# team-ergo-unipi/ergo_uvo

Hardware: AMD Instinct MI355X
Metric: stereo frame-pairs/sec (detect+match+pose) @1920x1080, 3k kpts (higher is better)
Workload: dtype f32+f64

## Files before the change

ergo_uvo_amd/csrc/surf.hip:

```cpp
#include "uvo_ctx.h"
#include <type_traits>
#include <string.h>
#include "uvo_math.h"
#include <algorithm>
#include <utility>
#include <vector>
#include <string>

namespace uvo {

struct ImgPair { const uint8_t* img[2]; int32_t* sum[2]; int32_t* planes[2]; int pw, pstride; int* cand_n; int* big_n; int* surv_n; };
struct AreaTab;
struct CandOut { uvo_keypoint* cand[2]; int* count; int cap; };
struct SurvOut { Survivor* list; int* count; int cap; };
static_assert(sizeof(Survivor) == 128, "a survivor record is 32 words");
struct SortArgs { const uvo_keypoint* cand[2]; const int* cand_n; uvo_keypoint* out[2]; int* out_n[2]; int* rank; int cap;
                  int4* big_par; int* big_n; int* gate_nqa; int gate_min_features; };
struct DescArgs { const uint8_t* img[2]; uvo_keypoint* kps[2]; float* desc[2]; const int* n[2]; const float* DW;
                  const int4* big_par; const int* big_n; const int* big_large; int cap;
                  const AreaTab* tabs; const int* iscale;
                  int extended;
                  const int32_t* sum[2]; const float* ori_w; int* ori_drop; };
struct LaneArgs { ImgPair ip; int32_t* part; SurvOut sv; CandOut out; SortArgs sa; DescArgs da; uint8_t* patch; const int4* big_in; int4* big_out; int* big_large; };
static const int kStripRows = 8;
// ... 707 lines not shown
    constexpr int QPR = OctTile<O, TW>::TWq / 4, kQuads = THs * QPR, kFill = UVO_FILL(kQuads, NT), kQ = NT / QPR, kR = NT % QPR;
    static_assert(STEP == 1 || STEP == 2, "tile fill handles octaves 0 and 1");
    static_assert(OctTile<O, TW>::TWq < kSumPad && STEP - OC::LO < kSumPad, "integral slack too small for the tile overshoot");
    int fidx = tid, fty = tid / QPR, fq = tid - fty * QPR;
#pragma unroll 1
    for (int i0 = 0; i0 < kQuads; i0 += NT * kFill) {
        SumQuad v[kFill];
        int dst[kFill];
#pragma unroll
        for (int u = 0; u < kFill; u++) {
            const bool in = fidx < kQuads;
            const int gy = min(max(sy0 + fty, 0), h), gx = sx0 + 4 * fq;
            v[u] = *reinterpret_cast<const SumQuad*>(gsum + (in ? gy * sw + gx : 0));
            dst[u] = in ? fty * STEP * PW + (4 / STEP) * fq : -1;
            fidx += NT; fq += kR; fty += kQ;
            if (fq >= QPR) { fq -= QPR; fty++; }
        }
#pragma unroll
        for (int u = 0; u < kFill; u++) {
            if (dst[u] < 0) continue;
            if constexpr (STEP == 1) {
                *reinterpret_cast<int4*>(stile + dst[u]) = make_int4(v[u].a, v[u].b, v[u].c, v[u].d);
            } else {
                *reinterpret_cast<int2*>(stile + dst[u]) = make_int2(v[u].a, v[u].c);
                *reinterpret_cast<int2*>(stile + dst[u] + PW) = make_int2(v[u].b, v[u].d);
            }
        }
    }
    nms_zero<TW, TH>(reinterpret_cast<unsigned*>(stile + THs * STEP * PW));
    __syncthreads();
    hess_stamp(1);
    det_layer_c<O, 1, TW, TH, NT>(stile, sdet, op, px0, py0, thr);
    det_layer_c<O, 2, TW, TH, NT>(stile, sdet, op, px0, py0, thr);
    det_layer_c<O, 3, TW, TH, NT>(stile, sdet, op, px0, py0, thr);
    __syncthreads();
    hess_stamp(2);
    nms_survivors<TW, TH, NT>(sdet, reinterpret_cast<unsigned*>(stile + THs * STEP * PW), op, thr, px0, py0, im, sv);
}
template <int O, int TW, int TH, int NT>
__global__ __launch_bounds__(NT) void k_hessian_nms_c(LaneArgs LA, int w, int h, OctavePat op, float thr)
{
    extern __shared__ __align__(16) unsigned char smem[];
    hessian_nms_c_tile<O, TW, TH, NT>(LA.ip, w, h, op, thr, LA.sv, blockIdx.x, blockIdx.y, blockIdx.z, smem);
}

template <int O, int TW, int TH, int NT>
__global__ __launch_bounds__(NT) void k_hessian_nms_p(LaneArgs LA, int w, int h, OctavePat op, float thr)
{
    __shared__ float sdet[3 * TH * TW];
    __shared__ unsigned s_list[NmsLds<TW, TH>::kWords];
    const ImgPair& ip = LA.ip; const SurvOut& sv = LA.sv;
    const int im = blockIdx.z;
    const int px0 = blockIdx.x * (TW - 2) - 1, py0 = blockIdx.y * (TH - 2) - 1;
    det_layer_p<O, 1, TW, TH, NT>(ip.planes[im], ip.pw, ip.pstride, sdet, op, px0, py0, thr);
    det_layer_p<O, 2, TW, TH, NT>(ip.planes[im], ip.pw, ip.pstride, sdet, op, px0, py0, thr);
    det_layer_p<O, 3, TW, TH, NT>(ip.planes[im], ip.pw, ip.pstride, sdet, op, px0, py0, thr);
    nms_zero<TW, TH>(s_list);
    __syncthreads();
    nms_survivors<TW, TH, NT>(sdet, s_list, op, thr, px0, py0, im, sv);
}

static const int kP23Threads = 512;
struct P23Grid { int nbx2, nb2, nbx3, nb3; };
template <class OP>
__device__ __forceinline__ void hessian_nms_p23_tile(const ImgPair& ip, const OP& op2, const OP& op3, float thr, const SurvOut& sv,
                                                     bool oct3, int bx, int by, int im, float* sdet, unsigned* s_list)
{
    constexpr int TW2 = 32, TH2 = 16, TW3 = 16, TH3 = 16;
    static_assert(TW3 * TH3 <= TW2 * TH2 && NmsLds<TW3, TH3>::kWords <= NmsLds<TW2, TH2>::kWords, "octave 3 reuses octave 2's LDS");
    if (!oct3) {
        const int px0 = bx * (TW2 - 2) - 1, py0 = by * (TH2 - 2) - 1;
        det_layers_p3<2, TW2, TH2, kP23Threads>(ip.planes[im], ip.pw, ip.pstride, sdet, op2, px0, py0, thr);
        nms_zero<TW2, TH2>(s_list);
        __syncthreads();
        hess_stamp(2);
        nms_survivors<TW2, TH2, kP23Threads>(sdet, s_list, op2, thr, px0, py0, im, sv);
    } else {
        const int px0 = bx * (TW3 - 2) - 1, py0 = by * (TH3 - 2) - 1;
        det_layers_p3<3, TW3, TH3, kP23Threads>(ip.planes[im], ip.pw, ip.pstride, sdet, op3, px0, py0, thr);
        nms_zero<TW3, TH3>(s_list);
        __syncthreads();
        hess_stamp(2);
        nms_survivors<TW3, TH3, kP23Threads>(sdet, s_list, op3, thr, px0, py0, im, sv);
    }
}
static const int kP23SdetFloats = 3 * 16 * 32;
static const int kO1TileRows = 18;
struct HessGrid { int nbx0, nb0, nbx1, nb1; P23Grid g; };
template <int TW, int TH>
__global__ __launch_bounds__(kP23Threads) void k_hessian_nms_all(LaneArgs LA, int w, int h, HessDims hd, float thr,
                                                                 const uint32_t* __restrict__ order)
{
    extern __shared__ __align__(16) unsigned char smem[];
    const ImgPair& ip = LA.ip;
    SurvOut sv = LA.sv;
    asm volatile("" : "+s"(sv.list), "+s"(sv.count), "+s"(sv.cap));
    const int im = blockIdx.y;
    const unsigned e = order[blockIdx.x];
    const int kind = e >> 30, bx = e & 0x3FFF, by = (e >> 14) & 0x3FFF;
    hess_stamp(0); hess_stamp(4, kind);
    if (kind == 0) hessian_nms_c_tile<0, TW, TH, kP23Threads>(ip, w, h, hd.o[0], thr, sv, bx, by, im, smem);
    else if (kind == 1) hessian_nms_c_tile<1, 32, kO1TileRows, kP23Threads>(ip, w, h, hd.o[1], thr, sv, bx, by, im, smem);
    else {
        float* sdet = reinterpret_cast<float*>(smem);
        hessian_nms_p23_tile(ip, hd.o[2], hd.o[3], thr, sv, kind == 3, bx, by, im, sdet, reinterpret_cast<unsigned*>(sdet + kP23SdetFloats));
    }
    hess_stamp(3);
}

__global__ __launch_bounds__(256) void k_probe_hold(int ticks)
{
    extern __shared__ int probe_lds[];
    if (threadIdx.x == 0) probe_lds[0] = ticks;
    const long long t0 = wall_clock64();
    while (wall_clock64() - t0 < ticks) __builtin_amdgcn_s_sleep(16);
}

__global__ void k_hessian_layer_debug(const int32_t* gsum, int w, int h, LayerPat lp, int step, int rows, int cols,
                                      float* det, float* trace)
{
    int j = blockIdx.x * blockDim.x + threadIdx.x, i = blockIdx.y;
    if (j >= lp.samples_j || i >= lp.samples_i) return;
    const int sw = w + 1;
    const int32_t* o = gsum + (size_t)(i * step) * sw + j * step;
    float dx, dy, dxy;
    haar_response(lp, [&](int yy, int xx) { return o[(size_t)yy * sw + xx]; }, &dx, &dy, &dxy);
    size_t pos = (size_t)(i + lp.margin) * cols + (j + lp.margin);
    det[pos] = dx * dy - 0.81f * dxy * dxy;
    trace[pos] = dx + dy;
}

__device__ __forceinline__ uint32_t ord_f32(float f)
{
    uint32_t b = __float_as_uint(f);
    return b ^ ((b >> 31) ? 0xFFFFFFFFu : 0x80000000u);
}
struct SortKey { unsigned long long k1, k2, k3; };
__device__ __forceinline__ SortKey make_sort_key(const uvo_keypoint& kp)
{
    SortKey k;
    k.k1 = ((unsigned long long)ord_f32(kp.response) << 32) | ord_f32(kp.size);
    k.k2 = ((unsigned long long)(uint32_t)kp.octave << 32) | ord_f32(kp.y);
    k.k3 = ((unsigned long long)(~ord_f32(kp.x)) << 32) | (uint32_t)(1 - kp.class_id);
    return k;
}

static const int kSmallWin = 128;
static const int kMaxWin = 740;
static const int kBigBins = 1024;
static const int kTripleWin = 246;
static const int kOrderThreads = 1024;
static const int kOrderPer = 8;
static const int kOrderCap = kOrderThreads * kOrderPer;
static const int kOrderBucketBits = 12;
static const int kOrderBuckets = 1 << kOrderBucketBits;
static const int kOrderBinsPer = kOrderBuckets / kOrderThreads;
static_assert(kOrderBuckets % kOrderThreads == 0 && kBigBins == kOrderThreads, "k_order scans kOrderBinsPer buckets and one window bin per thread");
static_assert(kOrderCap <= 65536, "bucket members are 16-bit candidate indices");

__global__ __launch_bounds__(1024) void k_big_sort(LaneArgs LA, int cap, const int* __restrict__ iscale_tab)
{
    const int4* __restrict__ in = LA.big_in; int4* __restrict__ out = LA.big_out; const int* __restrict__ big_n = LA.da.big_n; int* __restrict__ big_large = LA.big_large;
    const int im = blockIdx.x, tid = threadIdx.x;
    if (min(LA.sa.cand_n[im], cap) <= kOrderCap) return;
    const int n = min(big_n[im], cap);
    __shared__ int hist[kBigBins], scan[kBigBins];
    hist[tid] = 0;
    __syncthreads();
    for (int e = tid; e < n; e += 1024) atomicAdd(&hist[min(kBigBins - 1, max(0, kBigBins - 1 - in[im * cap + e].y))], 1);
    __syncthreads();
    int v = hist[tid];
    scan[tid] = v;
    __syncthreads();
    for (int off = 1; off < kBigBins; off <<= 1) {
        const int add = tid >= off ? scan[tid - off] : 0;
        __syncthreads();
        scan[tid] += add;
        __syncthreads();
    }
    hist[tid] = scan[tid] - v;
    if (tid == kBigBins - 1 - kTripleWin) big_large[im] = scan[tid] - v;
    __syncthreads();
    for (int e = tid; e < n; e += 1024) {
        int4 par = in[im * cap + e];
        const int pos = atomicAdd(&hist[min(kBigBins - 1, max(0, kBigBins - 1 - par.y))], 1);
        par.y |= iscale_tab[min(par.y, kMaxWin)] << 16;
        out[im * cap + pos] = par;
    }
}
static const int kSortChunk = 128;

__device__ __forceinline__ int wave_incl_scan(int v)
{
    const int lane = threadIdx.x & 63;
#pragma unroll
    for (int d = 1; d < 64; d <<= 1) { const int t = __shfl_up(v, d); if (lane >= d) v += t; }
    return v;
}

__global__ __launch_bounds__(kOrderThreads) void k_order(LaneArgs LA, const int* __restrict__ iscale_tab)
{
    const SortArgs& a = LA.sa;
    const int im = blockIdx.y, tid = threadIdx.x, lane = tid & 63, wv = tid >> 6;
    const int n = min(a.cand_n[im], a.cap);
    if (n > kOrderCap) return;
    __shared__ unsigned long long s_k1[kOrderCap];
    __shared__ unsigned short s_mem[kOrderCap];
    __shared__ int s_bin[kOrderBuckets];
    __shared__ int s_win[kBigBins];
    __shared__ int s_wave[2][kOrderThreads / 64];
    __shared__ unsigned s_lo, s_hi;
#pragma unroll
    for (int k = 0; k < kOrderBinsPer; k++) s_bin[tid * kOrderBinsPer + k] = 0;
    s_win[tid] = 0;
    if (tid == 0) { s_lo = 0xFFFFFFFFu; s_hi = 0; }
    __syncthreads();

    uvo_keypoint kp[kOrderPer];
    unsigned long long k1[kOrderPer];
    int wbin[kOrderPer];
    unsigned lo = 0xFFFFFFFFu, hi = 0;
#pragma unroll
    for (int k = 0; k < kOrderPer; k++) kp[k] = a.cand[im][min(k * kOrderThreads + tid, max(n - 1, 0))];
#pragma unroll
    for (int k = 0; k < kOrderPer; k++) {
        const int e = k * kOrderThreads + tid;
        wbin[k] = -1;
        k1[k] = make_sort_key(kp[k]).k1;
        if (e < n) {
            const unsigned r = ord_f32(kp[k].response);
            lo = min(lo, r); hi = max(hi, r);
            const float sc = kp[k].size * 1.2f / 9.0f;
            const int win_size = (int)((20 + 1) * sc);
            if (win_size > kSmallWin) { wbin[k] = min(kBigBins - 1, max(0, kBigBins - 1 - win_size)); atomicAdd(&s_win[wbin[k]], 1); }
        }
    }
#pragma unroll
    for (int d = 32; d > 0; d >>= 1) { lo = min(lo, (unsigned)__shfl_xor((int)lo, d)); hi = max(hi, (unsigned)__shfl_xor((int)hi, d)); }
    if (lane == 0) { atomicMin(&s_lo, lo); atomicMax(&s_hi, hi); }
    __syncthreads();

    lo = s_lo; hi = s_hi;
    const int bits = hi > lo ? 32 - __clz((int)(hi - lo)) : 0;
    const int sh = bits > kOrderBucketBits ? bits - kOrderBucketBits : 0;
    int bkt[kOrderPer];
#pragma unroll
    for (int k = 0; k < kOrderPer; k++) {
        const int e = k * kOrderThreads + tid;
        bkt[k] = -1;
        if (e < n) { bkt[k] = kOrderBuckets - 1 - (int)((ord_f32(kp[k].response) - lo) >> sh); atomicAdd(&s_bin[bkt[k]], 1); }
    }
    __syncthreads();

    int cnt[kOrderBinsPer], sb = 0;
#pragma unroll
    for (int k = 0; k < kOrderBinsPer; k++) { cnt[k] = s_bin[tid * kOrderBinsPer + k]; sb += cnt[k]; }
    const int wcnt = s_win[tid];
    const int ib = wave_incl_scan(sb), iw = wave_incl_scan(wcnt);
    if (lane == 63) { s_wave[0][wv] = ib; s_wave[1][wv] = iw; }
    __syncthreads();
    int xb = ib - sb, xw = iw - wcnt, wtot = 0;
    for (int v = 0; v < kOrderThreads / 64; v++) { if (v < wv) { xb += s_wave[0][v]; xw += s_wave[1][v]; } wtot += s_wave[1][v]; }
#pragma unroll
    for (int k = 0; k < kOrderBinsPer; k++) { s_bin[tid * kOrderBinsPer + k] = xb; xb += cnt[k]; }
    s_win[tid] = xw;
    if (tid == kBigBins - 1 - kTripleWin) LA.big_large[im] = xw;
    if (tid == 0) {
        a.big_n[im] = wtot;
        *a.out_n[im] = n;
        if (im == 0 && a.gate_nqa) {
            const int nL = n, nR = min(a.cand_n[1], a.cap);
            *a.gate_nqa = (nL >= a.gate_min_features && nR >= a.gate_min_features) ? nL : 0;
        }
    }
    __syncthreads();
    int slot[kOrderPer];
#pragma unroll
    for (int k = 0; k < kOrderPer; k++)
        if (bkt[k] >= 0) { slot[k] = atomicAdd(&s_bin[bkt[k]], 1); s_mem[slot[k]] = (unsigned short)(k * kOrderThreads + tid); s_k1[slot[k]] = k1[k]; }
    __syncthreads();

#pragma unroll
    for (int k = 0; k < kOrderPer; k++) {
        if (bkt[k] < 0) continue;
        const int e = k * kOrderThreads + tid;
        const int beg = bkt[k] > 0 ? s_bin[bkt[k] - 1] : 0, end = s_bin[bkt[k]];
        int rank = beg;
#pragma unroll 4
        for (int q = beg; q < end; q++) {
            const unsigned long long o1 = s_k1[q];
            rank += o1 > k1[k] ? 1 : 0;
            if (o1 == k1[k] && q != slot[k]) {
                const int f = s_mem[q];
                const SortKey mine = make_sort_key(kp[k]), o = make_sort_key(a.cand[im][f]);
                rank += (o.k2 > mine.k2 || (o.k2 == mine.k2 && (o.k3 > mine.k3 || (o.k3 == mine.k3 && f < e)))) ? 1 : 0;
            }
        }
        a.out[im][rank] = kp[k];
        if (wbin[k] >= 0) {
            const float sc = kp[k].size * 1.2f / 9.0f;
            const int win_size = (int)((20 + 1) * sc);
            const float win_offset = -(float)(win_size - 1) / 2;
            const int pos = atomicAdd(&s_win[wbin[k]], 1);
            LA.big_out[im * a.cap + pos] = make_int4(rank, win_size | (iscale_tab[min(win_size, kMaxWin)] << 16),
                                                     cv_round_f(kp[k].x + win_offset), cv_round_f(kp[k].y - win_offset));
        }
    }
}

__global__ __launch_bounds__(256) void k_rank_partial(LaneArgs LA)
{
    const SortArgs& a = LA.sa;
    const int im = blockIdx.y, tid = threadIdx.x;
    const int n = min(a.cand_n[im], a.cap);
    if (n <= kOrderCap) return;
    __shared__ SortKey tile[kSortChunk];
    __shared__ unsigned long long tile_k1[kSortChunk];
    const int nib = (n + 255) / 256, ntiles = nib * ((n + kSortChunk - 1) / kSortChunk);
    for (int t_ = blockIdx.x; t_ < ntiles; t_ += gridDim.x) {
        const int i0 = (t_ % nib) * 256, j0 = (t_ / nib) * kSortChunk;
        const int cnt = min(kSortChunk, n - j0);
        const int me = i0 + tid;
        uvo_keypoint mykp = {};
        if (me < n) mykp = a.cand[im][me];
        for (int t = tid; t < cnt; t += 256) { tile[t] = make_sort_key(a.cand[im][j0 + t]); tile_k1[t] = tile[t].k1; }
        __syncthreads();
        if (me < n) {
            const SortKey mine = make_sort_key(mykp);
            int rank = 0;
#pragma unroll 16
            for (int k = 0; k < cnt; k++) {
                const unsigned long long o1 = tile_k1[k];
                rank += o1 > mine.k1 ? 1 : 0;
                if (o1 == mine.k1) {
                    const SortKey o = tile[k];
                    rank += (o.k2 > mine.k2 || (o.k2 == mine.k2 && (o.k3 > mine.k3 || (o.k3 == mine.k3 && j0 + k < me)))) ? 1 : 0;
                }
            }
            atomicAdd(&a.rank[im * a.cap + me], rank);
        }
        __syncthreads();
    }
}

__global__ __launch_bounds__(256) void k_rank_scatter(LaneArgs LA)
{
    const SortArgs& a = LA.sa;
    const int im = blockIdx.y;
    const int n = min(a.cand_n[im], a.cap);
    if (n <= kOrderCap) return;
    const int me = blockIdx.x * 256 + threadIdx.x;
    bool big = false;
    int4 par = make_int4(0, 0, 0, 0);
    if (me < n) {
        int r = a.rank[im * a.cap + me];
        a.rank[im * a.cap + me] = 0;
        const uvo_keypoint kp = a.cand[im][me];
        a.out[im][r] = kp;
        const float sc = kp.size * 1.2f / 9.0f;
        const int win_size = (int)((20 + 1) * sc);
        if (win_size > kSmallWin) {
            const float win_offset = -(float)(win_size - 1) / 2;
            big = true;
            par = make_int4(r, win_size, cv_round_f(kp.x + win_offset), cv_round_f(kp.y - win_offset));
        }
    }
    {
        const int lane = threadIdx.x & 63;
        const unsigned long long m = __ballot(big);
        if (m != 0) {
            int base = 0;
            const int leader = __ffsll((long long)m) - 1;
            if (lane == leader) base = atomicAdd(&a.big_n[im], __popcll(m));
            base = __shfl(base, leader);
            if (big) a.big_par[im * a.cap + base + __popcll(m & ((1ull << lane) - 1))] = par;
        }
    }
    if (me == 0) *a.out_n[im] = n;
    if (me == 0 && im == 0 && a.gate_nqa) {
        const int nL = n, nR = min(a.cand_n[1], a.cap);
        *a.gate_nqa = (nL >= a.gate_min_features && nR >= a.gate_min_features) ? nL : 0;
    }
}

struct AreaTab { int sx1, sx2; float a_first, a_mid, a_last; bool has_first, has_last; };

__host__ __device__ __forceinline__ AreaTab area_tab(int dx, int ssize, double scale)
{
    AreaTab t;
    double fsx1 = dx * scale;
    double fsx2 = fsx1 + scale;
    double cellWidth = scale < ssize - fsx1 ? scale : ssize - fsx1;
    int sx1 = cv_ceil_d(fsx1), sx2 = cv_floor_d(fsx2);
    sx2 = sx2 < ssize - 1 ? sx2 : ssize - 1;
    sx1 = sx1 < sx2 ? sx1 : sx2;
    t.sx1 = sx1; t.sx2 = sx2;
    t.has_first = sx1 - fsx1 > 1e-3;
    t.a_first = (float)((sx1 - fsx1) / cellWidth);
    t.a_mid = (float)(1.0 / cellWidth);
    t.has_last = fsx2 - sx2 > 1e-3;
    double a = fsx2 - sx2; if (a > 1.) a = 1.; if (a > cellWidth) a = cellWidth;
    t.a_last = (float)(a / cellWidth);
    return t;
}

__device__ __forceinline__ uint8_t sat_u8(float v) { int iv = cv_round_f(v); return (uint8_t)(iv < 0 ? 0 : iv > 255 ? 255 : iv); }


__device__ __forceinline__ void describe_tail(const DescArgs& a, int im, int k, const int (*PATCH)[21])
{
    const int tid = threadIdx.x;
    __shared__ float DX[20][20], DY[20][20];
    __shared__ float vec[128];
    __shared__ float s_scale;
    const int dsize = a.extended ? 128 : 64;
    for (int o = tid; o < 400; o += 256) {
        int i = o / 20, j = o - i * 20;
        float dw = a.DW[o];
        float vx = (PATCH[i][j+1] - PATCH[i][j] + PATCH[i+1][j+1] - PATCH[i+1][j]) * dw;
        float vy = (PATCH[i+1][j] - PATCH[i][j] + PATCH[i+1][j+1] - PATCH[i][j+1]) * dw;
        DX[i][j] = vx; DY[i][j] = vy;
    }
    __syncthreads();
    if (tid < dsize) {
        float acc = 0.f;
        if (!a.extended) {
            int cell = tid >> 2, comp = tid & 3, ci = cell >> 2, cj = cell & 3;
            for (int y = ci * 5; y < ci * 5 + 5; y++)
                for (int x = cj * 5; x < cj * 5 + 5; x++) {
                    float t = (comp & 1) ? DY[y][x] : DX[y][x];
                    acc += (comp & 2) ? (float)fabs(t) : t;
                }
        } else {
            int cell = tid >> 3, comp = tid & 7, ci = cell >> 2, cj = cell & 3;
            for (int y = ci * 5; y < ci * 5 + 5; y++)
                for (int x = cj * 5; x < cj * 5 + 5; x++) {
                    const float tx = DX[y][x], ty = DY[y][x];
                    const float val = comp < 4 ? tx : ty, sel = comp < 4 ? ty : tx;
                    const bool take = (comp & 2) ? sel < 0 : sel >= 0;
                    if (take) acc += (comp & 1) ? (float)fabs(val) : val;
                }
        }
        vec[tid] = acc;
    }
    __syncthreads();
    if (tid == 0) {
        double square_mag = 0;
        for (int kk = 0; kk < dsize; kk++) square_mag += vec[kk] * vec[kk];
        s_scale = (float)(1. / (sqrt(square_mag) + FLT_EPSILON));
    }
    __syncthreads();
    if (tid < dsize) a.desc[im][(size_t)k * dsize + tid] = vec[tid] * s_scale;
}

static const int kTapBatch = 16;
__device__ long long* g_desc_stamps = nullptr;
__device__ __forceinline__ void desc_stamp(int im, int k, int slot, long long v = -1)
{
#if UVO_STAMPS
// ... 685 lines not shown

struct MergedGrid { int nbx0, nb0, nbx1, nb1, nb23, total; P23Grid g; };
static const int kMergedTW0 = 64, kMergedTH0 = 32, kMergedTW1 = 32;
static MergedGrid merged_grid(const OctavePat* ops)
{
    constexpr int TW0 = kMergedTW0, TH0 = kMergedTH0, TW1 = kMergedTW1, TH1 = kO1TileRows;
    MergedGrid m;
    m.nbx0 = (ops[0].cols + TW0 - 3) / (TW0 - 2); m.nb0 = m.nbx0 * ((ops[0].rows + TH0 - 3) / (TH0 - 2));
    m.nbx1 = (ops[1].cols + TW1 - 3) / (TW1 - 2); m.nb1 = m.nbx1 * ((ops[1].rows + TH1 - 3) / (TH1 - 2));
    m.g.nbx2 = (ops[2].cols + 32 - 3) / (32 - 2); m.g.nb2 = m.g.nbx2 * ((ops[2].rows + 16 - 3) / (16 - 2));
    m.g.nbx3 = (ops[3].cols + 16 - 3) / (16 - 2); m.g.nb3 = m.g.nbx3 * ((ops[3].rows + 16 - 3) / (16 - 2));
    m.nb23 = m.g.nb2 + m.g.nb3; m.total = m.nb0 + m.nb1 + m.nb23;
    return m;
}
static bool merged_launch(const Ctx* c)
{
    static const bool split_env = getenv("UVO_HESSIAN_SPLIT") != nullptr;
    return c->p.SURF_OCTAVES_NUMBER == 4 && !split_env;
}

uvo_status surf_prepare(Ctx* c, int w, int h)
{
    if (c->p.SURF_OCTAVES_NUMBER < 1 || c->p.SURF_OCTAVES_NUMBER > 4 || c->p.SURF_OCTAVES_LAYERS != 3) {
        c->err = "SURF: supported nOctaves 1..4, nOctaveLayers 3";
        return UVO_INVALID_ARG;
    }
    OctavePat ops[4];
    memset(ops, 0, sizeof(ops));
    for (int o = 0; o < c->p.SURF_OCTAVES_NUMBER; o++) make_octave(o, c->p.SURF_OCTAVES_LAYERS, w, h, &ops[o]);
    if (!c->d_octpat) UVO_HIP_TRY(c, hipMalloc(&c->d_octpat, sizeof(ops)));
    if (c->h_octpat.size() != sizeof(ops) || memcmp(c->h_octpat.data(), ops, sizeof(ops)) != 0) {
        UVO_HIP_TRY(c, hipStreamSynchronize(c->stream));
        c->h_octpat.assign(reinterpret_cast<const unsigned char*>(ops), reinterpret_cast<const unsigned char*>(ops) + sizeof(ops));
        UVO_HIP_TRY(c, hipMemcpyAsync(c->d_octpat, c->h_octpat.data(), sizeof(ops), hipMemcpyHostToDevice, c->stream));
        UVO_HIP_TRY(c, hipStreamSynchronize(c->stream));
    }
    if (!merged_launch(c)) return UVO_OK;
    const MergedGrid m = merged_grid(ops);
    const int nb0 = m.nb0, nb1 = m.nb1, nb23 = m.nb23, total = m.total;
    if (nb0 > 0x3FFF || nb1 > 0x3FFF || nb23 > 0x3FFF) { c->err = "SURF: image too large for the merged detection launch's tile table"; return UVO_INVALID_ARG; }
    const int ng[3] = { nb0, nb1, nb23 }, ngroups = total;
    if ((int)c->h_hess_order.size() != ngroups || c->hess_order_key[0] != nb0 || c->hess_order_key[1] != nb1 || c->hess_order_key[2] != nb23) {
        std::vector<std::pair<double, uint32_t>> pos;
        pos.reserve((size_t)ngroups);
        for (int k = 0; k < 3; k++) for (int i = 0; i < ng[k]; i++) {
            uint32_t e;
            if (k == 0) e = (0u << 30) | ((uint32_t)(i / m.nbx0) << 14) | (uint32_t)(i % m.nbx0);
            else if (k == 1) e = (1u << 30) | ((uint32_t)(i / m.nbx1) << 14) | (uint32_t)(i % m.nbx1);
            else if (i < m.g.nb2) e = (2u << 30) | ((uint32_t)(i / m.g.nbx2) << 14) | (uint32_t)(i % m.g.nbx2);
            else e = (3u << 30) | ((uint32_t)((i - m.g.nb2) / m.g.nbx3) << 14) | (uint32_t)((i - m.g.nb2) % m.g.nbx3);
            pos.emplace_back((i + 0.5) / ng[k] + k * 1e-9, e);
        }
        std::sort(pos.begin(), pos.end());
        c->h_hess_order.resize((size_t)ngroups);
        for (int b = 0; b < ngroups; b++) c->h_hess_order[(size_t)b] = pos[(size_t)b].second;
        UVO_HIP_TRY(c, hipStreamSynchronize(c->stream));
        if (c->d_hess_order_cap < (size_t)ngroups) {
            if (c->d_hess_order) (void)hipFree(c->d_hess_order);
            c->d_hess_order = nullptr; c->d_hess_order_cap = 0;
            UVO_HIP_TRY(c, hipMalloc(reinterpret_cast<void**>(&c->d_hess_order), sizeof(uint32_t) * (size_t)ngroups));
            c->d_hess_order_cap = (size_t)ngroups;
        }
        UVO_HIP_TRY(c, hipMemcpyAsync(c->d_hess_order, c->h_hess_order.data(), sizeof(uint32_t) * (size_t)ngroups, hipMemcpyHostToDevice, c->stream));
        UVO_HIP_TRY(c, hipStreamSynchronize(c->stream));
        c->hess_order_key[0] = nb0; c->hess_order_key[1] = nb1; c->hess_order_key[2] = nb23;
    }
    return UVO_OK;
}

uvo_status surf_detect(Ctx* c, int nimg, int gate_min_features)
{
    const int w = c->img_w, h = c->img_h;
    UVO_TRY(surf_prepare(c, w, h));
    const LaneArgs LA = lane_args(c, nimg, gate_min_features);
    UVO_TRY(surf_integral_launch(c, LA, nimg));
    const float thr = (float)c->p.SURF_MIN_HESSIAN;
    {
        OctavePat ops[4];
        memset(ops, 0, sizeof(ops));
        for (int o = 0; o < c->p.SURF_OCTAVES_NUMBER; o++) make_octave(o, c->p.SURF_OCTAVES_LAYERS, w, h, &ops[o]);
        const bool merged = merged_launch(c);
        if (merged) {
            constexpr int TW0 = kMergedTW0, TH0 = kMergedTH0, TW1 = kMergedTW1, TH1 = kO1TileRows;
            constexpr int THs0 = (TH0 - 1) * OctC<0>::STEP + (OctC<0>::HI - OctC<0>::LO) + 1, THs1 = (TH1 - 1) * OctC<1>::STEP + (OctC<1>::HI - OctC<1>::LO) + 1;
            constexpr size_t lds0 = sizeof(float) * 3 * TW0 * TH0 + sizeof(int32_t) * (size_t)THs0 * OctC<0>::STEP * OctTile<0, TW0>::PW + sizeof(unsigned) * NmsLds<TW0, TH0>::kWords;
            constexpr size_t lds1 = sizeof(float) * 3 * TW1 * TH1 + sizeof(int32_t) * (size_t)THs1 * OctC<1>::STEP * OctTile<1, TW1>::PW + sizeof(unsigned) * NmsLds<TW1, TH1>::kWords;
            constexpr size_t lds = lds0 > lds1 ? lds0 : lds1;
            static_assert(lds <= 54600, "three blocks of the merged detection launch must fit a CU's 160 KB of LDS");
            const MergedGrid mg = merged_grid(ops);
            const HessGrid hg = { mg.nbx0, mg.nb0, mg.nbx1, mg.nb1, mg.g };
            const int total = mg.total;
            auto kern = k_hessian_nms_all<TW0, TH0>;
            static bool attr_dev[64] = {false};
            bool& attr_set = attr_dev[c->device & 63];
            if (!attr_set) { UVO_HIP_TRY(c, hipFuncSetAttribute(reinterpret_cast<const void*>(kern), hipFuncAttributeMaxDynamicSharedMemorySize, (int)lds)); attr_set = true; }
            StageTimer t(c, ST_HESSIAN_O0);
            static const size_t lds_pad = getenv("UVO_HESS_LDS") ? (size_t)atoi(getenv("UVO_HESS_LDS")) : 0;
            const size_t lds_launch = lds_pad > lds ? lds_pad : lds;
            if (lds_pad > lds) { static bool once = false; if (!once) { (void)hipFuncSetAttribute(reinterpret_cast<const void*>(kern), hipFuncAttributeMaxDynamicSharedMemorySize, (int)lds_launch); once = true; } }
            static const char* stamps_path = UVO_STAMPS ? getenv("UVO_HESS_STAMPS") : nullptr;
            static long long* d_stamps = nullptr; static size_t stamps_n = 0;
            if (stamps_path && c->lane_id == 0) {
                if (!d_stamps) { stamps_n = (size_t)total * 4 * 8; (void)hipMalloc(reinterpret_cast<void**>(&d_stamps), sizeof(long long) * stamps_n); (void)hipMemcpyToSymbol(HIP_SYMBOL(g_hess_stamps), &d_stamps, sizeof(d_stamps)); }
                (void)hipMemsetAsync(d_stamps, 0, sizeof(long long) * stamps_n, c->stream);
            }
            HessDims hd;
            for (int o = 0; o < 4; o++) {
                OctDims& d = hd.o[o];
                for (int l = 0; l < 5; l++) { d.L[l].samples_i = ops[o].L[l].samples_i; d.L[l].samples_j = ops[o].L[l].samples_j; }
                d.rows = ops[o].rows; d.cols = ops[o].cols; d.octave = ops[o].octave;
                for (int l = 0; l < 3; l++) d.nms_margin[l] = ops[o].nms_margin[l];
            }
            Ctx::TraceRec* trh = (c->trace_on && c->trace_cur >= 0) ? &c->trace[c->trace_cur] : nullptr;
            if (trh) (void)hipEventRecord(trh->ev[6], c->stream);
            hipLaunchKernelGGL(kern, dim3(total, nimg), dim3(kP23Threads), lds_launch, c->stream, LA, w, h, hd, thr, c->d_hess_order);
            if (trh) { (void)hipEventRecord(trh->ev[7], c->stream); trh->det_marked = true; }
            if (stamps_path && d_stamps && c->lane_id == 0) {
                std::vector<long long> hs(stamps_n);
                (void)hipStreamSynchronize(c->stream);
                (void)hipMemcpy(hs.data(), d_stamps, sizeof(long long) * stamps_n, hipMemcpyDeviceToHost);
                if (FILE* f = fopen(stamps_path, "w")) {
                    fprintf(f, "block,im,kind,t_start,t_filled,t_det,t_end,t_scan,t_scanbar,t_atomic\n");
                    for (int y = 0; y < nimg; y++) for (int b = 0; b < total; b++) { const long long* r = hs.data() + ((size_t)y * total + b) * 8; fprintf(f, "%d,%d,%lld,%lld,%lld,%lld,%lld,%lld,%lld,%lld\n", b, y, r[4], r[0], r[1], r[2], r[3], r[5], r[6], r[7]); }
                    fclose(f);
                }
            }
            UVO_HIP_TRY(c, hipGetLastError());
        }
        for (int o = 0; o < c->p.SURF_OCTAVES_NUMBER && !merged; o++) {
            StageTimer t(c, ST_HESSIAN_O0 + o);
            const OctavePat& op = ops[o];
            hipError_t e;
            if (o == 0)      e = launch_hessian_c<0, 64, 24, 512>(c, LA, nimg, op, thr);
            else if (o == 1) e = launch_hessian_c<1, 32, 24, 512>(c, LA, nimg, op, thr);
            else if (o == 2) e = launch_hessian_p<2, 32, 16, 512>(c, LA, nimg, op, thr);
            else             e = launch_hessian_p<3, 16, 16, 256>(c, LA, nimg, op, thr);
            UVO_HIP_TRY(c, e);
        }
        {
            StageTimer t(c, ST_HESSIAN_O0 + c->p.SURF_OCTAVES_NUMBER - 1);
            hipLaunchKernelGGL(k_hessian_finish, dim3((c->surv_cap + kFinishPerWg - 1) / kFinishPerWg), dim3(256), 0, c->stream, LA, static_cast<const OctavePat*>(c->d_octpat), w, h);
            UVO_HIP_TRY(c, hipGetLastError());
        }
        static const int probe_thin = getenv("UVO_PROBE_THIN_US") ? atoi(getenv("UVO_PROBE_THIN_US")) : 0, probe_fat = getenv("UVO_PROBE_FAT_US") ? atoi(getenv("UVO_PROBE_FAT_US")) : 0;
        if (probe_thin > 0) hipLaunchKernelGGL(k_probe_hold, dim3(1), dim3(64), 64, c->stream, probe_thin * 100);
        if (probe_fat > 0) {
            static bool once = false;
            if (!once) { (void)hipFuncSetAttribute(reinterpret_cast<const void*>(k_probe_hold), hipFuncAttributeMaxDynamicSharedMemorySize, 53000); once = true; }
            hipLaunchKernelGGL(k_probe_hold, dim3(768), dim3(256), 53000, c->stream, probe_fat * 100);
        }
    }
    {
        StageTimer t(c, ST_SORT);
        hipLaunchKernelGGL(k_order, dim3(1, nimg), dim3(kOrderThreads), 0, c->stream, LA, c->d_area_iscale);
        if (c->cap > kOrderCap) {
            const int tiles_max = ((c->cap + 255) / 256) * ((c->cap + kSortChunk - 1) / kSortChunk);
            hipLaunchKernelGGL(k_rank_partial, dim3(tiles_max < 512 ? tiles_max : 512, nimg), dim3(256), 0, c->stream, LA);
            hipLaunchKernelGGL(k_rank_scatter, dim3((c->cap + 255) / 256, nimg), dim3(256), 0, c->stream, LA);
            hipLaunchKernelGGL(k_big_sort, dim3(nimg), dim3(1024), 0, c->stream, LA, c->cap, c->d_area_iscale);
        }
        UVO_HIP_TRY(c, hipGetLastError());
    }
    {
        StageTimer t(c, ST_DESCRIPTOR);
        const size_t lds_small = sizeof(float) * 21 * ((kSmallWin + 3) | 1), lds_big = sizeof(float) * 4 * kBigRow;
        if (c->p.SURF_UPRIGHT) {
            const int nbig = 1024;
            static const int desc_part = getenv("UVO_DESC_PART") ? atoi(getenv("UVO_DESC_PART")) : 0;
            static const char* dstamps_path = UVO_STAMPS ? getenv("UVO_DESC_STAMPS") : nullptr;
            static long long* d_dstamps = nullptr; const size_t dstamps_n = (size_t)4 * 16384 * 8;
            const bool dstamp = dstamps_path && c->lane_id == 0 && nimg == 2;
            if (dstamp) {
                if (!d_dstamps) { (void)hipMalloc(reinterpret_cast<void**>(&d_dstamps), sizeof(long long) * dstamps_n); (void)hipMemcpyToSymbol(HIP_SYMBOL(g_desc_stamps), &d_dstamps, sizeof(d_dstamps)); }
                (void)hipMemsetAsync(d_dstamps, 0, sizeof(long long) * dstamps_n, c->stream);
            }
            static const int fixed_grid = getenv("UVO_DESC_GRID") ? atoi(getenv("UVO_DESC_GRID")) : 0;
            const int hint = c->sh->kp_hint;
            int nsmall = hint > 0 ? ((hint + hint / 4 + 255) & ~255) : c->cap;
            if (fixed_grid != 0) nsmall = fixed_grid < 0 ? c->cap : fixed_grid;
            nsmall = nsmall < 512 ? 512 : (nsmall > c->cap ? c->cap : nsmall);
            static const int desc_order = getenv("UVO_DESC_ORDER") ? atoi(getenv("UVO_DESC_ORDER")) : 2;
            static const int nbig_env = getenv("UVO_DESC_NBIG") ? atoi(getenv("UVO_DESC_NBIG")) : 0;
            const int nbig_l = nbig_env > 0 ? nbig_env : nbig;
            hipLaunchKernelGGL(k_descriptor64, dim3((nbig_l + nsmall) * nimg), dim3(256), lds_small > lds_big ? lds_small : lds_big, c->stream, DescLane{ { LA } }, w, h, nbig_l, desc_part, nimg, desc_order);
            if (dstamp && d_dstamps) {
                std::vector<long long> hs(dstamps_n);
                (void)hipStreamSynchronize(c->stream);
                (void)hipMemcpy(hs.data(), d_dstamps, sizeof(long long) * dstamps_n, hipMemcpyDeviceToHost);
                if (FILE* f = fopen(dstamps_path, "w")) {
                    fprintf(f, "im,k,t_start,t_kp,t_ready,t_horiz,t_vert,t_end,win,kind\n");
                    for (int y = 0; y < 2; y++) for (int k = 0; k < 16384; k++) { const long long* r = hs.data() + ((size_t)y * 16384 + k) * 8; if (r[0]) fprintf(f, "%d,%d,%lld,%lld,%lld,%lld,%lld,%lld,%lld,%lld\n", y, k, r[0], r[1], r[2], r[3], r[4], r[5], r[6], r[7]); }
                    fclose(f);
                }
                if (FILE* f = fopen((std::string(dstamps_path) + ".big").c_str(), "w")) {
                    fprintf(f, "im,task,t_start,t_horiz,t_end,win,kind\n");
                    for (int y = 0; y < 2; y++) for (int k = 0; k < 16384; k++) { const long long* r = hs.data() + ((size_t)(2 + y) * 16384 + k) * 8; if (r[0] && r[2]) fprintf(f, "%d,%d,%lld,%lld,%lld,%lld,%lld\n", y, k, r[0], r[1], r[2], r[6], r[7]); }
                    fclose(f);
                }
            }
            hipLaunchKernelGGL(k_descriptor64_big_finish, dim3(1024, nimg), dim3(256), 0, c->stream, LA);
        } else {
            const DescArgs& da = LA.da;
            const size_t lds_rot = sizeof(float) * 21 * (kMaxWin + 1);
            static bool rot_attr_dev[64] = {false};
            bool& rot_attr = rot_attr_dev[c->device & 63];
            if (!rot_attr) { UVO_HIP_TRY(c, hipFuncSetAttribute(reinterpret_cast<const void*>(k_descriptor_rot), hipFuncAttributeMaxDynamicSharedMemorySize, (int)lds_rot)); rot_attr = true; }
            hipLaunchKernelGGL(k_surf_orientation, dim3((c->cap + 3) / 4, nimg), dim3(256), 0, c->stream, da, w, h);
            hipLaunchKernelGGL(k_descriptor_rot, dim3(2048, nimg), dim3(256), lds_rot, c->stream, da, w, h);
        }
        UVO_HIP_TRY(c, hipGetLastError());
    }
    return UVO_OK;
}

uvo_status surf_hessian_layer_debug(Ctx* c, int octave, int layer, float* det, float* trace)
{
    const int w = c->img_w, h = c->img_h;
    if (octave < 0 || octave > 3 || layer < 0 || layer > 4 || w <= 0) { c->err = "hessian_layer: bad octave/layer or no image"; return UVO_INVALID_ARG; }
    OctavePat op;
    make_octave(octave, 3, w, h, &op);
    size_t n = (size_t)op.rows * op.cols;
    float *d_det = nullptr, *d_tr = nullptr;
    UVO_HIP_TRY(c, hipMalloc(&d_det, sizeof(float) * n * 2));
    d_tr = d_det + n;
    UVO_HIP_TRY(c, hipMemsetAsync(d_det, 0, sizeof(float) * n * 2, c->stream));
    const LayerPat& lp = op.L[layer];
    if (lp.samples_i > 0) {
        dim3 g((lp.samples_j + 255) / 256, lp.samples_i);
        hipLaunchKernelGGL(k_hessian_layer_debug, g, dim3(256), 0, c->stream, c->d_sum[0], w, h, lp, op.step, op.rows, op.cols, d_det, d_tr);
    }
    UVO_HIP_TRY(c, hipMemcpyAsync(det, d_det, sizeof(float) * n, hipMemcpyDeviceToHost, c->stream));
    UVO_HIP_TRY(c, hipMemcpyAsync(trace, d_tr, sizeof(float) * n, hipMemcpyDeviceToHost, c->stream));
    UVO_HIP_TRY(c, hipStreamSynchronize(c->stream));
    (void)hipFree(d_det);
    return UVO_OK;
}

}
```

Baseline: 4033.

## Split keypoint ordering across workgroups with packed 16-bit bucket counters

The single-workgroup-per-image ordering kernel becomes a multi-workgroup kernel (default two per image). Each workgroup rebuilds the response histogram, then ranks only its own contiguous slice of response buckets. Bucket counts are packed as 16-bit halves, and the 64-bit key array is replaced by 32-bit words that hold the low response bits plus the candidate index, which shrinks LDS use and allows higher occupancy. Each workgroup rereads candidate fields through buffer loads instead of holding them in registers, so the histogram work is duplicated per group and global traffic increases.

Result: no change. 4047 (median of 6 runs) (+0.3%).

```diff
diff --git a/ergo_uvo_amd/csrc/surf.hip b/ergo_uvo_amd/csrc/surf.hip
--- a/ergo_uvo_amd/csrc/surf.hip
+++ b/ergo_uvo_amd/csrc/surf.hip
@@ -883,11 +883,15 @@
 static const int kOrderThreads = 1024;
 static const int kOrderPer = 8;
 static const int kOrderCap = kOrderThreads * kOrderPer;
+static const int kOrderIdxBits = 13;
 static const int kOrderBucketBits = 12;
 static const int kOrderBuckets = 1 << kOrderBucketBits;
 static const int kOrderBinsPer = kOrderBuckets / kOrderThreads;
-static_assert(kOrderBuckets % kOrderThreads == 0 && kBigBins == kOrderThreads, "k_order scans kOrderBinsPer buckets and one window bin per thread");
-static_assert(kOrderCap <= 65536, "bucket members are 16-bit candidate indices");
+static const int kOrderWinPer = kBigBins / kOrderThreads;
+static const int kOrderGrid = 2;
+static const size_t kOrderLdsBytes = sizeof(unsigned) * (kOrderCap + kOrderBuckets / 2 + kBigBins + kOrderThreads / 64 + 4);
+static_assert(kOrderBuckets % (2 * kOrderThreads) == 0 && kBigBins % kOrderThreads == 0, "k_order scans whole bucket words and window bins per thread");
+static_assert(kOrderCap == 1 << kOrderIdxBits && kOrderCap < 65536, "candidate indices fill kOrderIdxBits; counts and starts fit 16-bit halves");
 
 __global__ __launch_bounds__(1024) void k_big_sort(LaneArgs LA, int cap, const int* __restrict__ iscale_tab)
 {
@@ -929,42 +933,41 @@
     return v;
 }
 
-__global__ __launch_bounds__(kOrderThreads) void k_order(LaneArgs LA, const int* __restrict__ iscale_tab)
+__global__ __launch_bounds__(kOrderThreads) __attribute__((amdgpu_waves_per_eu(8, 8))) void k_order(LaneArgs LA, const int* __restrict__ iscale_tab)
 {
     const SortArgs& a = LA.sa;
-    const int im = blockIdx.y, tid = threadIdx.x, lane = tid & 63, wv = tid >> 6;
+    const int im = blockIdx.y, g = blockIdx.x, G = gridDim.x, tid = threadIdx.x, lane = tid & 63, wv = tid >> 6;
     const int n = min(a.cand_n[im], a.cap);
     if (n > kOrderCap) return;
-    __shared__ unsigned long long s_k1[kOrderCap];
-    __shared__ unsigned short s_mem[kOrderCap];
-    __shared__ int s_bin[kOrderBuckets];
-    __shared__ int s_win[kBigBins];
-    __shared__ int s_wave[2][kOrderThreads / 64];
-    __shared__ unsigned s_lo, s_hi;
-#pragma unroll
-    for (int k = 0; k < kOrderBinsPer; k++) s_bin[tid * kOrderBinsPer + k] = 0;
-    s_win[tid] = 0;
-    if (tid == 0) { s_lo = 0xFFFFFFFFu; s_hi = 0; }
-    __syncthreads();
-
-    uvo_keypoint kp[kOrderPer];
-    unsigned long long k1[kOrderPer];
-    int wbin[kOrderPer];
+    extern __shared__ unsigned order_lds[];
+    unsigned* const s_mem = order_lds;
+    unsigned* const s_bin = s_mem + kOrderCap;
+    unsigned* const s_win = s_bin + kOrderBuckets / 2;
+    int* const s_wave = reinterpret_cast<int*>(s_win + kBigBins);
+    unsigned* const s_cut = s_win + kBigBins + kOrderThreads / 64;
+    unsigned& s_lo = s_cut[2];
+    unsigned& s_hi = s_cut[3];
+    const uvo_keypoint* __restrict__ cand = a.cand[im];
+#pragma unroll
+    for (int k = 0; k < kOrderBinsPer / 2; k++) s_bin[k * kOrderThreads + tid] = 0;
+#pragma unroll
+    for (int k = 0; k < kOrderWinPer; k++) s_win[k * kOrderThreads + tid] = 0;
+    if (tid == 0) { s_lo = 0xFFFFFFFFu; s_hi = 0; s_cut[0] = s_cut[1] = ((unsigned)kOrderBuckets << 16) | (unsigned)n; }
+    __syncthreads();
+
     unsigned lo = 0xFFFFFFFFu, hi = 0;
-#pragma unroll
-    for (int k = 0; k < kOrderPer; k++) kp[k] = a.cand[im][min(k * kOrderThreads + tid, max(n - 1, 0))];
-#pragma unroll
-    for (int k = 0; k < kOrderPer; k++) {
-        const int e = k * kOrderThreads + tid;
-        wbin[k] = -1;
-        k1[k] = make_sort_key(kp[k]).k1;
-        if (e < n) {
-            const unsigned r = ord_f32(kp[k].response);
-            lo = min(lo, r); hi = max(hi, r);
-            const float sc = kp[k].size * 1.2f / 9.0f;
-            const int win_size = (int)((20 + 1) * sc);
-            if (win_size > kSmallWin) { wbin[k] = min(kBigBins - 1, max(0, kBigBins - 1 - win_size)); atomicAdd(&s_win[wbin[k]], 1); }
-        }
+    const int nv = (n - tid + kOrderThreads - 1) / kOrderThreads;
+    const __amdgpu_buffer_rsrc_t crs = __builtin_amdgcn_make_buffer_rsrc(const_cast<uvo_keypoint*>(cand), 0, max(n, 1) * (int)sizeof(uvo_keypoint), 0x00020000);
+    const int last_off = max(n - 1, 0) * (int)sizeof(uvo_keypoint), tid_off = tid * (int)sizeof(uvo_keypoint);
+    const int group_off = kOrderThreads * (int)sizeof(uvo_keypoint);
+    auto load_field = [&](int k, int field_off) { return __uint_as_float(__builtin_amdgcn_raw_buffer_load_b32(crs, min(k * group_off + tid_off, last_off) + field_off, 0, 0)); };
+    for (int k0 = 0; k0 * kOrderThreads < n; k0 += kOrderPer) {
+        unsigned r[kOrderPer];
+#pragma unroll
+        for (int k = 0; k < kOrderPer; k++) r[k] = ord_f32(load_field(k0 + k, (int)offsetof(uvo_keypoint, response)));
+#pragma unroll
+        for (int k = 0; k < kOrderPer; k++)
+            if (k0 + k < nv) { lo = min(lo, r[k]); hi = max(hi, r[k]); }
     }
 #pragma unroll
     for (int d = 32; d > 0; d >>= 1) { lo = min(lo, (unsigned)__shfl_xor((int)lo, d)); hi = max(hi, (unsigned)__shfl_xor((int)hi, d)); }
@@ -974,68 +977,140 @@
     lo = s_lo; hi = s_hi;
     const int bits = hi > lo ? 32 - __clz((int)(hi - lo)) : 0;
     const int sh = bits > kOrderBucketBits ? bits - kOrderBucketBits : 0;
-    int bkt[kOrderPer];
-#pragma unroll
-    for (int k = 0; k < kOrderPer; k++) {
-        const int e = k * kOrderThreads + tid;
-        bkt[k] = -1;
-        if (e < n) { bkt[k] = kOrderBuckets - 1 - (int)((ord_f32(kp[k].response) - lo) >> sh); atomicAdd(&s_bin[bkt[k]], 1); }
-    }
-    __syncthreads();
-
-    int cnt[kOrderBinsPer], sb = 0;
-#pragma unroll
-    for (int k = 0; k < kOrderBinsPer; k++) { cnt[k] = s_bin[tid * kOrderBinsPer + k]; sb += cnt[k]; }
-    const int wcnt = s_win[tid];
-    const int ib = wave_incl_scan(sb), iw = wave_incl_scan(wcnt);
-    if (lane == 63) { s_wave[0][wv] = ib; s_wave[1][wv] = iw; }
-    __syncthreads();
-    int xb = ib - sb, xw = iw - wcnt, wtot = 0;
-    for (int v = 0; v < kOrderThreads / 64; v++) { if (v < wv) { xb += s_wave[0][v]; xw += s_wave[1][v]; } wtot += s_wave[1][v]; }
-#pragma unroll
-    for (int k = 0; k < kOrderBinsPer; k++) { s_bin[tid * kOrderBinsPer + k] = xb; xb += cnt[k]; }
-    s_win[tid] = xw;
-    if (tid == kBigBins - 1 - kTripleWin) LA.big_large[im] = xw;
-    if (tid == 0) {
-        a.big_n[im] = wtot;
-        *a.out_n[im] = n;
-        if (im == 0 && a.gate_nqa) {
-            const int nL = n, nR = min(a.cand_n[1], a.cap);
-            *a.gate_nqa = (nL >= a.gate_min_features && nR >= a.gate_min_features) ? nL : 0;
-        }
-    }
-    __syncthreads();
-    int slot[kOrderPer];
-#pragma unroll
-    for (int k = 0; k < kOrderPer; k++)
-        if (bkt[k] >= 0) { slot[k] = atomicAdd(&s_bin[bkt[k]], 1); s_mem[slot[k]] = (unsigned short)(k * kOrderThreads + tid); s_k1[slot[k]] = k1[k]; }
-    __syncthreads();
-
-#pragma unroll
-    for (int k = 0; k < kOrderPer; k++) {
-        if (bkt[k] < 0) continue;
-        const int e = k * kOrderThreads + tid;
-        const int beg = bkt[k] > 0 ? s_bin[bkt[k] - 1] : 0, end = s_bin[bkt[k]];
+    const int drop = max(0, sh - (32 - kOrderIdxBits));
+    for (int k0 = 0; k0 * kOrderThreads < n; k0 += kOrderPer) {
+        unsigned r[kOrderPer];
+#pragma unroll
+        for (int k = 0; k < kOrderPer; k++) r[k] = ord_f32(load_field(k0 + k, (int)offsetof(uvo_keypoint, response)));
+#pragma unroll
+        for (int k = 0; k < kOrderPer; k++)
+            if (k0 + k < nv) {
+                const int b = kOrderBuckets - 1 - (int)((r[k] - lo) >> sh);
+                atomicAdd(&s_bin[b >> 1], 1u << ((b & 1) * 16));
+            }
+    }
+    __syncthreads();
+
+    unsigned key0 = 0xFFFFFFFFu, key1 = 0xFFFFFFFFu;
+    {
+        unsigned wd[kOrderBinsPer / 2];
+        int sb = 0;
+#pragma unroll
+        for (int k = 0; k < kOrderBinsPer / 2; k++) { wd[k] = s_bin[tid * (kOrderBinsPer / 2) + k]; sb += (int)(wd[k] & 0xFFFFu) + (int)(wd[k] >> 16); }
+        const int ib = wave_incl_scan(sb);
+        if (lane == 63) s_wave[wv] = ib;
+        __syncthreads();
+        unsigned xb = (unsigned)(ib - sb);
+        for (int v = 0; v < wv; v++) xb += (unsigned)s_wave[v];
+        const unsigned cut0 = (unsigned)g * (unsigned)n, cut1 = cut0 + (unsigned)n;
+#pragma unroll
+        for (int k = 0; k < kOrderBinsPer; k++) {
+            const unsigned b = (unsigned)(tid * kOrderBinsPer + k);
+            if (xb * (unsigned)G >= cut0) key0 = min(key0, (b << 16) | xb);
+            if (xb * (unsigned)G >= cut1) key1 = min(key1, (b << 16) | xb);
+            const unsigned cnt = (k & 1) ? wd[k >> 1] >> 16 : wd[k >> 1] & 0xFFFFu;
+            wd[k >> 1] = (k & 1) ? (wd[k >> 1] & 0xFFFFu) | (xb << 16) : (wd[k >> 1] & 0xFFFF0000u) | xb;
+            xb += cnt;
+        }
+#pragma unroll
+        for (int k = 0; k < kOrderBinsPer / 2; k++) s_bin[tid * (kOrderBinsPer / 2) + k] = wd[k];
+#pragma unroll
+        for (int d = 32; d > 0; d >>= 1) { key0 = min(key0, (unsigned)__shfl_xor((int)key0, d)); key1 = min(key1, (unsigned)__shfl_xor((int)key1, d)); }
+        if (lane == 0) { atomicMin(&s_cut[0], key0); atomicMin(&s_cut[1], key1); }
+    }
+    __syncthreads();
+    const int b0 = (int)(s_cut[0] >> 16), b1 = (int)(s_cut[1] >> 16);
+    const int base = (int)(s_cut[0] & 0xFFFFu), m = (int)(s_cut[1] & 0xFFFFu) - base;
+
+    for (int k0 = 0; k0 * kOrderThreads < n; k0 += kOrderPer) {
+        unsigned r[kOrderPer];
+        float sz[kOrderPer];
+#pragma unroll
+        for (int k = 0; k < kOrderPer; k++) {
+            r[k] = ord_f32(load_field(k0 + k, (int)offsetof(uvo_keypoint, response)));
+            sz[k] = load_field(k0 + k, (int)offsetof(uvo_keypoint, size));
+        }
+#pragma unroll
+        for (int k = 0; k < kOrderPer; k++) {
+            const int e = (k0 + k) * kOrderThreads + tid;
+            if (k0 + k >= nv) continue;
+            const unsigned d = r[k] - lo;
+            const int b = kOrderBuckets - 1 - (int)(d >> sh);
+            const float sc = sz[k] * 1.2f / 9.0f;
+            const int win_size = (int)((20 + 1) * sc);
+            if (win_size > kSmallWin) atomicAdd(&s_win[min(kBigBins - 1, max(0, kBigBins - 1 - win_size))], 1u + (b < b0 ? 0x10000u : 0u));
+            if (b >= b0 && b < b1) {
+                const int hs = (b & 1) * 16;
+                const int slot = (int)((atomicAdd(&s_bin[b >> 1], 1u << hs) >> hs) & 0xFFFFu) - base;
+                s_mem[slot] = (((d & ((1u << sh) - 1u)) >> drop) << kOrderIdxBits) | (unsigned)e;
+            }
+        }
+    }
+    __syncthreads();
+
+    {
+        unsigned ww[kOrderWinPer];
+        int sw = 0;
+#pragma unroll
+        for (int k = 0; k < kOrderWinPer; k++) { ww[k] = s_win[tid * kOrderWinPer + k]; sw += (int)(ww[k] & 0xFFFFu); }
+        const int iw = wave_incl_scan(sw);
+        if (lane == 63) s_wave[wv] = iw;
+        __syncthreads();
+        int xw = iw - sw, wtot = 0;
+        for (int v = 0; v < kOrderThreads / 64; v++) { if (v < wv) xw += s_wave[v]; wtot += s_wave[v]; }
+#pragma unroll
+        for (int k = 0; k < kOrderWinPer; k++) {
+            const int bin = tid * kOrderWinPer + k;
+            s_win[bin] = (unsigned)xw + (ww[k] >> 16);
+            if (g == 0 && bin == kBigBins - 1 - kTripleWin) LA.big_large[im] = xw;
+            xw += (int)(ww[k] & 0xFFFFu);
+        }
+        if (g == 0 && tid == 0) {
+            a.big_n[im] = wtot;
+            *a.out_n[im] = n;
+            if (im == 0 && a.gate_nqa) {
+                const int nL = n, nR = min(a.cand_n[1], a.cap);
+                *a.gate_nqa = (nL >= a.gate_min_features && nR >= a.gate_min_features) ? nL : 0;
+            }
+        }
+    }
+    __syncthreads();
+
+    int q = tid;
+    unsigned w = 0;
+    uvo_keypoint kp = {};
+    if (q < m) { w = s_mem[q]; kp = cand[w & (kOrderCap - 1)]; }
+    while (q < m) {
+        const int qn = q + kOrderThreads;
+        unsigned wn = 0;
+        uvo_keypoint kpn = {};
+        if (qn < m) { wn = s_mem[qn]; kpn = cand[wn & (kOrderCap - 1)]; }
+        const int e = (int)(w & (kOrderCap - 1));
+        const unsigned pre = w >> kOrderIdxBits;
+        const int b = kOrderBuckets - 1 - (int)((ord_f32(kp.response) - lo) >> sh);
+        const int beg = b > b0 ? (int)((s_bin[(b - 1) >> 1] >> (((b - 1) & 1) * 16)) & 0xFFFFu) : base;
+        const int end = (int)((s_bin[b >> 1] >> ((b & 1) * 16)) & 0xFFFFu);
         int rank = beg;
 #pragma unroll 4
-        for (int q = beg; q < end; q++) {
-            const unsigned long long o1 = s_k1[q];
-            rank += o1 > k1[k] ? 1 : 0;
-            if (o1 == k1[k] && q != slot[k]) {
-                const int f = s_mem[q];
-                const SortKey mine = make_sort_key(kp[k]), o = make_sort_key(a.cand[im][f]);
-                rank += (o.k2 > mine.k2 || (o.k2 == mine.k2 && (o.k3 > mine.k3 || (o.k3 == mine.k3 && f < e)))) ? 1 : 0;
-            }
-        }
-        a.out[im][rank] = kp[k];
-        if (wbin[k] >= 0) {
-            const float sc = kp[k].size * 1.2f / 9.0f;
-            const int win_size = (int)((20 + 1) * sc);
+        for (int p = beg - base; p < end - base; p++) {
+            const unsigned o = s_mem[p];
+            rank += (o >> kOrderIdxBits) > pre ? 1 : 0;
+            if ((o >> kOrderIdxBits) == pre && p != q) {
+                const int f = (int)(o & (kOrderCap - 1));
+                const SortKey mine = make_sort_key(kp), ok = make_sort_key(cand[f]);
+                rank += (ok.k1 > mine.k1 || (ok.k1 == mine.k1 && (ok.k2 > mine.k2 || (ok.k2 == mine.k2 && (ok.k3 > mine.k3 || (ok.k3 == mine.k3 && f < e)))))) ? 1 : 0;
+            }
+        }
+        a.out[im][rank] = kp;
+        const float sc = kp.size * 1.2f / 9.0f;
+        const int win_size = (int)((20 + 1) * sc);
+        if (win_size > kSmallWin) {
             const float win_offset = -(float)(win_size - 1) / 2;
-            const int pos = atomicAdd(&s_win[wbin[k]], 1);
+            const int pos = (int)atomicAdd(&s_win[min(kBigBins - 1, max(0, kBigBins - 1 - win_size))], 1u);
             LA.big_out[im * a.cap + pos] = make_int4(rank, win_size | (iscale_tab[min(win_size, kMaxWin)] << 16),
-                                                     cv_round_f(kp[k].x + win_offset), cv_round_f(kp[k].y - win_offset));
-        }
+                                                     cv_round_f(kp.x + win_offset), cv_round_f(kp.y - win_offset));
+        }
+        q = qn; w = wn; kp = kpn;
     }
 }
 
@@ -2027,7 +2102,8 @@
     }
     {
         StageTimer t(c, ST_SORT);
-        hipLaunchKernelGGL(k_order, dim3(1, nimg), dim3(kOrderThreads), 0, c->stream, LA, c->d_area_iscale);
+        static const int order_grid = getenv("UVO_ORDER_GRID") ? std::min(std::max(atoi(getenv("UVO_ORDER_GRID")), 1), 64) : kOrderGrid;
+        hipLaunchKernelGGL(k_order, dim3(order_grid, nimg), dim3(kOrderThreads), kOrderLdsBytes, c->stream, LA, c->d_area_iscale);
         if (c->cap > kOrderCap) {
             const int tiles_max = ((c->cap + 255) / 256) * ((c->cap + kSortChunk - 1) / kSortChunk);
             hipLaunchKernelGGL(k_rank_partial, dim3(tiles_max < 512 ? tiles_max : 512, nimg), dim3(256), 0, c->stream, LA);
```
